# duanzhiihao/myDetection

Measured on AMD Instinct MI355X. Metric: images/sec at batch 32, 640x640, YOLOv3-80 (backbone -> FPN -> head -> decode -> NMS), higher is better.
Workload: dtype f32; 1 GPU; yolov3_80 (Darknet-53 + YOLOv3 FPN/head + decode + conf 0.005/top-512/NMS 0.45), batch 32/GPU, 640x640, random-init calibrated weights, hipGraph replay (1 batch lane per GPU); global_batch=32, image_size=640, parallelism=dp1, batch_lanes=1, batch_lanes_rule=model.batch_lanes_hint, passes=153, exchange=none

## Files before the change

include/mydet.h:

```cpp
#ifndef MYDET_H
#define MYDET_H

#include <stdint.h>

#ifdef __cplusplus
extern "C" {
#endif

#define MYDET_ABI_VERSION 2

#define MYDET_E_BADARG   (-1)
#define MYDET_E_UNSUPP   (-2)

#define MYDET_ACT_NONE   0
#define MYDET_ACT_LEAKY  1
#define MYDET_ACT_SWISH  2

int mydet_abi_version(void);

int mydet_conv2d_igemm_f32(const float *x, int64_t ldx, const float *w,
                           const float *scale, const float *shift,
                           const float *residual, int64_t ldr, const float *a_gate,
                           void *workspace, int64_t workspace_bytes,
                           float *y, int64_t ldy,
// ... 25 lines not shown
int mydet_dwconv_se_groups(int Ho, int Wo, int C, int K, int stride);
int mydet_dwconv_f32(const float *x, int64_t ldx, const float *w, const float *scale, const float *shift,
                     float *y, int64_t ldy, int B, int H, int W, int C, int K, int stride, int pad_t, int pad_l,
                     int Ho, int Wo, int act, float *se_partial, int S, const mydet_se_tail *se, void *stream);

int mydet_channel_sums_f32(const float *x, int64_t ldx, int B, int H, int W, int C, float *partial, int S,
                           void *stream);

int mydet_se_gate_f32(float *partial, int S, int B, int HW, int C, const float *w1, const float *b1, int Cse,
                      const float *w2t, const float *b2, float *gate, void *stream);

int mydet_maxpool3s2_f32(const float *x, int64_t ldx, float *y, int64_t ldy, int B, int H, int W, int C,
                         int Ho, int Wo, void *stream);

int mydet_bifpn_fuse_f32(int n, const float *in0, int64_t ld0, int mode0, const float *in1, int64_t ld1, int mode1,
                         const float *in2, int64_t ld2, int mode2, const float *weights, float *y, int64_t ldy,
                         int B, int H, int W, int C, void *stream);

int mydet_upsample_concat_f32(const float *a, int64_t lda, int Ha, int Wa, int C1,
                              const float *b, int64_t ldb, int C2,
                              float *y, int64_t ldy, int B, int Ho, int Wo, void *stream);

int mydet_conv1x1_upcat_f32(const float *x_lo, int64_t ld_lo, int C_lo, const float *x_hi, int64_t ld_hi, int C_hi,
                            const float *w, const float *scale, const float *shift, void *workspace,
                            int64_t workspace_bytes, float *y, int64_t ldy, int B, int H, int W, int Cout, int act,
                            void *stream);

int64_t mydet_split_bf16_elems(int Cout, int K);
int mydet_split_bf16_f32(const float *w, int Cout, int K, uint16_t *planes, void *stream);
int mydet_conv2d_igemm_b3_f32(const float *x, int64_t ldx, const uint16_t *w_planes, const float *scale, const float *shift,
                              const float *residual, int64_t ldr, const float *a_gate, void *workspace, int64_t workspace_bytes, float *y,
                              int64_t ldy, int B, int H, int W, int Cin, int Cout, int KH, int KW, int stride, int pad_t,
                              int pad_l, int Ho, int Wo, int act, void *stream);
int mydet_conv3x3_p3_f32(const float *x, int64_t ldx, const uint16_t *w_planes, const float *scale, const float *shift,
                         const float *residual, int64_t ldr, float *y, int64_t ldy, int B, int H, int W, int Cin, int Cout,
                         int stride, int act, void *stream);
int mydet_conv3x3_p3_plan(int Ho, int Wo, int Cout, int stride, int32_t *out);
int mydet_conv_stem_p3_f32(const float *x, int64_t sxb, int64_t sxc, int64_t sxh, int64_t sxw, const uint16_t *w0_planes,
                           const float *scale0, const float *shift0, int act0, const uint16_t *w1_planes, const float *scale1,
                           const float *shift1, int act1, float *y, int64_t ldy, int B, int H, int W, int C0, int Cout,
                           int stride0, int pad_t, int pad_l, int Hs, int Ws, int stride1, void *stream);
int mydet_conv_stem_p3_lds_bytes(void);
int mydet_conv_b3_reload_tuning(void);

int mydet_conv_igemm_occupancy(int cfg, int *assumed);

int mydet_conv_igemm_plan(int cfg, int B, int Ho, int Wo, int Cin, int Cout, int taps,
                          int64_t workspace_bytes, int cus, int32_t *out);

int mydet_space_to_depth_f32(const float *x, int64_t sb, int64_t sc, int64_t sh, int64_t sw, float *y, int64_t ldy,
                             int B, int C, int H, int W, void *stream);

int mydet_spp_concat_f32(const float *x, int64_t ldx, float *y, int64_t ldy, int B, int H, int W, int C, int k0, int k1,
                         int k2, void *stream);

#define MYDET_DECODE_YOLO   0
#define MYDET_DECODE_RETINA 1
#define MYDET_DECODE_FCOS   2
#define MYDET_DECODE_RAPID  3
typedef struct mydet_decode_level {
    const float *box; int64_t ldbox;
    const float *cls; int64_t ldcls;
    const float *anchors_wh;
    int H, W;
    float stride;
    int64_t n_off;
// ... 179 lines not shown
```

mydetection_amd/_lib.py:

```python
import ctypes
import os

_HERE = os.path.dirname(os.path.abspath(__file__))
LIB_PATH = os.environ.get('MYDET_LIB_PATH') or os.path.join(_HERE, 'lib', 'libmydet_hip.so')

c_int, c_i64, c_f32, c_f64, c_ptr = ctypes.c_int, ctypes.c_int64, ctypes.c_float, ctypes.c_double, ctypes.c_void_p

SIGNATURES = {
    'mydet_abi_version': [],
    'mydet_conv2d_igemm_f32': [c_ptr, c_i64, c_ptr, c_ptr, c_ptr, c_ptr, c_i64, c_ptr, c_ptr, c_i64, c_ptr, c_i64]
    + [c_int] * 13 + [c_ptr],
    'mydet_wino_weights_floats': [c_int, c_int],
    'mydet_wino_weights_f32': [c_ptr, c_int, c_int, c_ptr, c_ptr],
    'mydet_conv2d_wino_f32': [c_ptr, c_i64, c_ptr, c_ptr, c_ptr, c_ptr, c_i64, c_ptr, c_i64, c_ptr, c_i64] + [c_int] * 6
    + [c_ptr],
    'mydet_wino4_weights_floats': [c_int, c_int],
    'mydet_wino4_weights_f32': [c_ptr, c_int, c_int, c_ptr, c_ptr],
    'mydet_wino4_workspace_bytes': [c_int, c_int, c_int, c_int, c_int],
    'mydet_wino4_reload_tuning': [],
    'mydet_conv_b3_reload_tuning': [],
    'mydet_conv_igemm_occupancy': [c_int, c_ptr],
    'mydet_conv_igemm_plan': [c_int] * 7 + [c_i64, c_int, c_ptr],
    'mydet_split_bf16_elems': [c_int, c_int],
    'mydet_split_bf16_f32': [c_ptr, c_int, c_int, c_ptr, c_ptr],
    'mydet_conv2d_igemm_b3_f32': [c_ptr, c_i64, c_ptr, c_ptr, c_ptr, c_ptr, c_i64, c_ptr, c_ptr, c_i64, c_ptr, c_i64] + [c_int] * 13 + [c_ptr],
    'mydet_conv3x3_p3_f32': [c_ptr, c_i64, c_ptr, c_ptr, c_ptr, c_ptr, c_i64, c_ptr, c_i64] + [c_int] * 7 + [c_ptr],
    'mydet_conv3x3_p3_plan': [c_int, c_int, c_int, c_int, c_ptr],
    'mydet_conv_stem_p3_f32': [c_ptr, c_i64, c_i64, c_i64, c_i64, c_ptr, c_ptr, c_ptr, c_int, c_ptr, c_ptr, c_ptr, c_int, c_ptr, c_i64]
    + [c_int] * 11 + [c_ptr],
    'mydet_conv_stem_p3_lds_bytes': [],
    'mydet_wino4_tail_plan': [c_int, c_int, c_int, c_int, c_int, c_int, c_ptr],
    'mydet_conv2d_wino4_f32': [c_ptr, c_i64, c_ptr, c_ptr, c_ptr, c_ptr, c_i64, c_ptr, c_i64, c_ptr, c_i64] + [c_int] * 6 + [c_ptr],
    'mydet_dwconv_slices': [c_int, c_int, c_int, c_int, c_int],
    'mydet_dwconv_se_groups': [c_int, c_int, c_int, c_int, c_int],
    'mydet_dwconv_f32': [c_ptr, c_i64, c_ptr, c_ptr, c_ptr, c_ptr, c_i64] + [c_int] * 11 + [c_ptr, c_int, c_ptr, c_ptr],
    'mydet_channel_sums_f32': [c_ptr, c_i64, c_int, c_int, c_int, c_int, c_ptr, c_int, c_ptr],
    'mydet_se_gate_f32': [c_ptr, c_int, c_int, c_int, c_int, c_ptr, c_ptr, c_int, c_ptr, c_ptr, c_ptr, c_ptr],
    'mydet_maxpool3s2_f32': [c_ptr, c_i64, c_ptr, c_i64] + [c_int] * 6 + [c_ptr],
    'mydet_bifpn_fuse_f32': [c_int, c_ptr, c_i64, c_int, c_ptr, c_i64, c_int, c_ptr, c_i64, c_int, c_ptr, c_ptr, c_i64,
                             c_int, c_int, c_int, c_int, c_ptr],
    'mydet_conv2d_stem_f32': [c_ptr, c_i64, c_i64, c_i64, c_i64, c_ptr, c_ptr, c_ptr, c_ptr, c_i64] + [c_int] * 10 + [c_ptr],
    'mydet_upsample_concat_f32': [c_ptr, c_i64, c_int, c_int, c_int, c_ptr, c_i64, c_int, c_ptr, c_i64, c_int, c_int,
                                  c_int, c_ptr],
    'mydet_conv1x1_upcat_f32': [c_ptr, c_i64, c_int, c_ptr, c_i64, c_int, c_ptr, c_ptr, c_ptr, c_ptr, c_i64, c_ptr, c_i64]
    + [c_int] * 5 + [c_ptr],
    'mydet_space_to_depth_f32': [c_ptr, c_i64, c_i64, c_i64, c_i64, c_ptr, c_i64, c_int, c_int, c_int, c_int, c_ptr],
    'mydet_spp_concat_f32': [c_ptr, c_i64, c_ptr, c_i64] + [c_int] * 7 + [c_ptr],
    'mydet_decode_levels_f32': [c_int, c_int, c_ptr, c_int, c_int, c_int, c_int, c_int, c_int, c_int, c_int, c_int, c_int,
                                c_ptr, c_ptr, c_ptr, c_i64, c_ptr],
    'mydet_decode_uv5_levels_f32': [c_int, c_ptr, c_int, c_int, c_int, c_int, c_int, c_int, c_int, c_int, c_int, c_int,
                                    c_ptr, c_ptr, c_ptr, c_i64, c_ptr],
    'mydet_decode_f32': [c_int, c_ptr, c_i64, c_int, c_int, c_ptr, c_i64, c_int, c_int, c_int, c_ptr, c_int, c_int,
                         c_int, c_int, c_int, c_f32, c_int, c_int, c_ptr, c_ptr, c_ptr, c_i64, c_i64, c_ptr],
    'mydet_postprocess_f32': [c_ptr, c_ptr, c_ptr, c_int, c_i64, c_f32, c_f64, c_int, c_ptr, c_ptr, c_ptr, c_ptr,
                              c_ptr, c_ptr, c_ptr],
    'mydet_postprocess_records_f32': [c_ptr, c_ptr, c_ptr, c_int, c_i64, c_f32, c_f64, c_ptr, c_ptr, c_ptr],
    'mydet_postprocess_rot_f32': [c_ptr, c_ptr, c_ptr, c_int, c_i64, c_f32, c_f64, c_int, c_ptr, c_ptr, c_ptr, c_ptr,
                                  c_ptr, c_ptr, c_ptr],
    'mydet_postprocess_records_rot_f32': [c_ptr, c_ptr, c_ptr, c_int, c_i64, c_f32, c_f64, c_ptr, c_ptr, c_ptr],
    'mydet_postprocess_rotnms_f32': [c_ptr, c_ptr, c_ptr, c_int, c_i64, c_f32, c_f64, c_int, c_ptr, c_ptr, c_ptr, c_ptr,
                                     c_ptr, c_ptr, c_ptr],
    'mydet_postprocess_records_rotnms_f32': [c_ptr, c_ptr, c_ptr, c_int, c_i64, c_f32, c_f64, c_ptr, c_ptr, c_ptr],
    'mydet_rotated_iou_f32': [c_ptr, c_i64, c_ptr, c_i64, c_ptr, c_ptr],
    'mydet_mbconv_tiles': [c_int, c_int, c_int],
    'mydet_mbconv_expand_dw_f32': [c_ptr, c_i64, c_ptr, c_ptr, c_ptr, c_ptr, c_ptr, c_i64] + [c_int] * 11 + [c_ptr, c_int, c_ptr, c_ptr],
    'mydet_sepconv_nodes_f32': [c_int, c_ptr, c_int, c_int, c_ptr],
    'mydet_stem_dw_f32': [c_ptr, c_i64, c_i64, c_i64, c_i64, c_ptr, c_ptr, c_ptr, c_ptr, c_ptr, c_i64, c_int, c_int, c_int, c_int,
                          c_int, c_int, c_int, c_int, c_ptr, c_int, c_ptr, c_ptr],
    'mydet_lr_tb_levels_f32': [c_int, c_ptr, c_int, c_int, c_ptr],
    'mydet_sepconv_decode_retina_f32': [c_int, c_ptr, c_int, c_int, c_int, c_int, c_int, c_int, c_ptr, c_ptr, c_ptr, c_i64, c_ptr],
    'mydet_bboxes_iou_f32': [c_ptr, c_int, c_ptr, c_int, c_int, c_ptr, c_ptr],
    'mydet_bboxes_to_original_batched_f32': [c_ptr, c_i64, c_ptr, c_i64, c_int, c_int, c_ptr, c_ptr],
    'mydet_detections_to_json_f64': [c_ptr, c_i64, c_ptr, c_i64, c_ptr, c_i64, c_ptr, c_i64, c_int, c_int, c_ptr, c_int, c_ptr, c_ptr, c_ptr],
    'mydet_resize_bilinear_u8': [c_ptr, c_int, c_int, c_i64, c_ptr, c_int, c_int, c_i64, c_ptr, c_ptr, c_int, c_ptr, c_ptr, c_int, c_ptr],
    'mydet_preprocess_u8_f32': [c_ptr, c_int, c_int, c_int, c_ptr, c_int, c_int, c_int, c_ptr, c_ptr, c_ptr],
    'mydet_frames_to_input_f32': [c_ptr, c_int, c_int, c_int, c_i64, c_i64, c_ptr, c_int, c_int, c_int, c_int, c_int, c_int,
                                  c_ptr, c_ptr, c_int, c_ptr, c_ptr, c_int, c_int, c_ptr, c_ptr, c_ptr],
# ... 107 lines not shown
```

mydetection_amd/csrc/conv_igemm.hip:

```cpp
#include <cstdlib>

#include "common.h"
#include "split_bf16.h"

namespace {

constexpr unsigned OOB = 0xFFFFFFFFu;

struct ConvArgs {
    const float *x, *w, *scale, *shift, *res, *gate;
    float *y;
    int64_t ldx, ldr, ldy;
    int B, H, W, Cin, Cout, KH, KW, stride, pad_t, pad_l, Ho, Wo, act;
    int M, K, ntiles, nblk;
    int tile0, splits;
    float *ws;
    size_t ws_bytes;
    const float *x1;
    int64_t ldx1;
    int C1;
    const unsigned short *wsplit;
};

typedef unsigned u32x4 __attribute__((ext_vector_type(4)));
// ... 231 lines not shown
            store_slab(buf ^ 1, areg[d], breg[d]);
            load_slab(kt + d + 1 + PF, areg[d], breg[d]);
            __syncthreads();
            buf ^= 1;
        }
    }

    if (SPLIT) {
        constexpr int NV4 = TM * TN * 4;
        f32x4 *dst = reinterpret_cast<f32x4 *>(p.ws) + (int64_t)blockIdx.x * NV4 * NT + tid;
#pragma unroll
        for (int i = 0; i < TM; ++i)
#pragma unroll
            for (int j = 0; j < TN; ++j)
#pragma unroll
                for (int v = 0; v < 4; ++v)
                    dst[((i * TN + j) * 4 + v) * NT] =
                        f32x4{acc[i][j][4 * v], acc[i][j][4 * v + 1], acc[i][j][4 * v + 2], acc[i][j][4 * v + 3]};
        return;
    }
    const int m_base = m0 + wm * TM * 32, n_base = n0 + wn * TN * 32;
    if ((m0 + BM <= p.M) && (n0 + BN <= p.Cout))
        epilogue<ACT, RES, true, TM, TN>(p, acc, m_base, n_base, fr, fh, pscl, psft);
    else
        epilogue<ACT, RES, false, TM, TN>(p, acc, m_base, n_base, fr, fh, pscl, psft);
}

constexpr int B3_COUT_PAD = 256;
__device__ __host__ __forceinline__ int b3_unit(int rr, int h) { return 2 * rr + (h ^ ((rr >> 2) & 1)); }

#ifndef B3_PF
#define B3_PF 2
#endif
template <int BM, int BN, int ACT, bool RES, bool SPLIT = false, int PF = B3_PF, int WN = 2, bool GATE = false>
__global__ __launch_bounds__(128 * WN, 2) void conv_igemm_b3_kernel(const ConvArgs p) {
    constexpr int NT = 128 * WN, WM = 2, BK = 16;
    constexpr int ROWB = 32;
    constexpr int TM = BM / (WM * 32), TN = BN / (WN * 32);
    constexpr int AI = BM * 4 / NT;
    constexpr int BCH = BN * 2;
    constexpr int PLANE_A = BM * ROWB, PLANE_B = BN * ROWB, BUF = 3 * (PLANE_A + PLANE_B);
    extern __shared__ __attribute__((aligned(16))) char smem_b3[];

    const int tid = threadIdx.x;
    const int lid = SPLIT ? p.tile0 + (int)blockIdx.x / p.splits : mydet_xcd_remap(blockIdx.x, p.nblk);
    const int m0 = (lid / p.ntiles) * BM;
    const int n0 = (lid % p.ntiles) * BN;
    const int hwo = p.Ho * p.Wo;
    const int b0 = m0 / hwo;
    const int64_t img = (int64_t)p.H * p.W * p.ldx;
    const __amdgpu_buffer_rsrc_t xr = mydet_rsrc(p.x + b0 * img, (p.B - b0) * img * 4);
    const int CoutP = (p.Cout + B3_COUT_PAD - 1) / B3_COUT_PAD * B3_COUT_PAD;
    const __amdgpu_buffer_rsrc_t wr = mydet_rsrc(p.wsplit, (int64_t)((p.K + 15) >> 4) * 3 * CoutP * 32);

    constexpr int RP = NT / 4;
    const int sc = tid & 3, sr = tid >> 2;
    const int ntaps = p.KH * p.KW;
    int aoff[AI];
    unsigned amask[AI];
    unsigned goff[AI];
    const __amdgpu_buffer_rsrc_t gr = mydet_rsrc(GATE ? p.gate : p.x, (int64_t)p.B * p.Cin * 4);
    const bool flat = ntaps == 1 && p.stride == 1 && p.pad_t == 0 && p.pad_l == 0 && p.Ho == p.H && p.Wo == p.W;
#pragma unroll
    for (int i = 0; i < AI; ++i) {
        const int m = m0 + sr + RP * i;
        const int mm = m < p.M ? m : p.M - 1;
        goff[i] = GATE ? (unsigned)((mm / hwo) * p.Cin + sc * 4) * 4u : 0u;
        if (flat) {
            aoff[i] = (int)(((int64_t)(mm - b0 * hwo) * p.ldx + sc * 4) * 4);
            amask[i] = m < p.M ? 1u : 0u;
            continue;
        }
        const int ow = mm % p.Wo, t = mm / p.Wo;
        const int oh = t % p.Ho, b = t / p.Ho;
        const int ih0 = oh * p.stride - p.pad_t, iw0 = ow * p.stride - p.pad_l;
        aoff[i] = (int)((((int64_t)(b - b0) * p.H + ih0) * p.W + iw0) * p.ldx + sc * 4) * 4;
        unsigned mask = 0;
        for (int tp = 0; tp < ntaps; ++tp) {
            const int kh = tp / p.KW, kw = tp - kh * p.KW;
            if ((unsigned)(ih0 + kh) < (unsigned)p.H && (unsigned)(iw0 + kw) < (unsigned)p.W) mask |= 1u << tp;
        }
        amask[i] = m < p.M ? mask : 0u;
    }
    const bool bact = tid < BCH;
    const int bu = tid & 63, brr = bu >> 1;
    const int br = (tid >> 6) * 32 + brr, bh = (bu & 1) ^ ((brr >> 2) & 1);
    const unsigned boff = bact ? (unsigned)(n0 * 32 + tid * 16) : OOB;
    const unsigned plane_bytes = (unsigned)CoutP * 32u, slab_bytes = 3u * plane_bytes;

    f32x4 areg[PF][AI];
    u32x4 breg[PF][3];
    const int nk_all = (p.K + BK - 1) / BK;
    int kt0 = 0, nk = nk_all;
    if (SPLIT) {
        const int sp = (int)blockIdx.x % p.splits;
        kt0 = (int)((unsigned)(nk_all * sp) / (unsigned)p.splits);
        nk = (int)((unsigned)(nk_all * (sp + 1)) / (unsigned)p.splits);
    }
    int tap = 0, c0 = 0, tapoff = 0;
    if (SPLIT) {
        const int k0 = kt0 * BK;
        tap = k0 / p.Cin;
        c0 = k0 - tap * p.Cin;
        const int kh = tap / p.KW, kw = tap - kh * p.KW;
        tapoff = (int)(((int64_t)kh * p.W + kw) * p.ldx) * 4;
    }
    auto load_slab = [&](int kt, f32x4 (&ar)[AI], u32x4 (&brg)[3]) {
        const unsigned uoff = (unsigned)(tapoff + c0 * 4);
#pragma unroll
        for (int i = 0; i < AI; ++i) {
            bool ok = ((amask[i] >> tap) & 1u) && c0 + sc * 4 < p.Cin;
            ar[i] = buf_load16(xr, ok ? (unsigned)aoff[i] + uoff : OOB);
            if (GATE) {
                const f32x4 gv = buf_load16(gr, ok ? goff[i] + (unsigned)c0 * 4u : OOB);
#pragma unroll
                for (int e = 0; e < 4; ++e) ar[i][e] *= gv[e];
            }
        }
        c0 += BK;
        if (c0 == p.Cin) {
            c0 = 0;
            ++tap;
            const int kh = tap / p.KW, kw = tap - kh * p.KW;
            tapoff = (int)(((int64_t)kh * p.W + kw) * p.ldx) * 4;
        }
#pragma unroll
        for (int pl = 0; pl < 3; ++pl)
            brg[pl] = __builtin_amdgcn_raw_buffer_load_b128(wr, kt < nk_all ? boff : OOB,
                                                            __builtin_amdgcn_readfirstlane((unsigned)kt * slab_bytes + (unsigned)pl * plane_bytes), 0);
    };
    auto store_slab = [&](int buf, const f32x4 (&ar)[AI], const u32x4 (&brg)[3]) {
        char *a = smem_b3 + buf * BUF, *b = a + 3 * PLANE_A;
#pragma unroll
        for (int i = 0; i < AI; ++i) {
            bf16x4 q0, q1, q2;
            split3(ar[i], q0, q1, q2);
            char *d = a + (sr + RP * i) * ROWB + (((sc >> 1) ^ ((sr >> 3) & 1)) * 16) + (sc & 1) * 8;
            *reinterpret_cast<bf16x4 *>(d) = q0;
            *reinterpret_cast<bf16x4 *>(d + PLANE_A) = q1;
            *reinterpret_cast<bf16x4 *>(d + 2 * PLANE_A) = q2;
        }
        if (bact) {
#pragma unroll
            for (int pl = 0; pl < 3; ++pl) *reinterpret_cast<u32x4 *>(b + pl * PLANE_B + br * ROWB + ((bh ^ ((br >> 3) & 1)) * 16)) = brg[pl];
        }
// ... 420 lines not shown
    const TilePlan pl = plan_tiles(a.M, a.Cout, a.K, BM, BN, BK, slots, a0.ws ? a0.ws_bytes : 0);
    a.ntiles = pl.ntiles;
    const int total = pl.total, rem = pl.rem, splits = pl.splits;
    const bool split = pl.split;
    const size_t lds = (size_t)2 * (BM + BN) * (BK + 4) * sizeof(float);
    const bool cin = (a.Cin % BK) == 0;
    a.tile0 = 0; a.splits = 1;
    a.nblk = split ? total - rem : total;
    int rc = 0;
    if (a.x1) {
        if (!(BM == 64 && BN == 64 && BK == 32) || !cin || a.act != MYDET_ACT_LEAKY || a.res || a.gate) return MYDET_E_UNSUPP;
        if (a.nblk > 0) rc = launch_inst<64, 64, 2, 2, 32, true, MYDET_ACT_LEAKY, false, false, false, true>(a, lds, stream);
        if (rc || !split) return rc;
        a.tile0 = total - rem; a.splits = splits; a.nblk = rem * splits;
        rc = launch_inst<64, 64, 2, 2, 32, true, MYDET_ACT_NONE, false, false, true, true>(a, lds, stream);
        if (rc) return rc;
        return launch_fixup_act<BM, BN, WM, WN>(a, rem, stream);
    }
    if (a.nblk > 0)
        rc = cin ? launch_act<BM, BN, WM, WN, BK, true>(a, lds, stream) : launch_act<BM, BN, WM, WN, BK, false>(a, lds, stream);
    if (rc || !split) return rc;
    a.tile0 = total - rem; a.splits = splits; a.nblk = rem * splits;
    if (a.gate) {
        if (cin) rc = launch_inst<BM, BN, WM, WN, BK, true, MYDET_ACT_NONE, false, true, true>(a, lds, stream);
        else rc = launch_inst<BM, BN, WM, WN, BK, false, MYDET_ACT_NONE, false, true, true>(a, lds, stream);
    } else {
        if (cin) rc = launch_inst<BM, BN, WM, WN, BK, true, MYDET_ACT_NONE, false, false, true>(a, lds, stream);
        else rc = launch_inst<BM, BN, WM, WN, BK, false, MYDET_ACT_NONE, false, false, true>(a, lds, stream);
    }
    if (rc) return rc;
    return launch_fixup_act<BM, BN, WM, WN>(a, rem, stream);
}

template <int BM, int BN, int ACT, bool RES, bool SPLIT, int PF = B3_PF, int WN = 2, bool GATE = false>
int launch_b3_inst(const ConvArgs &a, hipStream_t stream) {
    auto kern = &conv_igemm_b3_kernel<BM, BN, ACT, RES, SPLIT, PF, WN, GATE>;
    constexpr int lds = 2 * 3 * (BM + BN) * 32;
    static unsigned long long attr_set = 0;
    if (const int e = mydet_lds_opt_in(attr_set, kern, lds)) return e;
    hipLaunchKernelGGL(kern, dim3(a.nblk), dim3(128 * WN), lds, stream, a);
    return mydet_launch_status();
}

template <int BM, int BN, int WN = 2>
int launch_b3(const ConvArgs &a0, hipStream_t stream) {
    ConvArgs a = a0;
    const int slots = 2 * mydet_cu_count();
    const int mtiles = (a.M + BM - 1) / BM;
    a.ntiles = (a.Cout + BN - 1) / BN;
    const int total = mtiles * a.ntiles;
    const int nk = (a.K + 15) / 16;
    const int rounds = total / slots;
    const int rem = total % slots;
    const bool small = rounds == 0 && total * 4 <= slots && nk >= 32;
    int splits = rem > 0 ? slots / rem : 0;
    if (splits > 16) splits = 16;
    if (splits > nk / 8) splits = nk / 8;
    const size_t need = (size_t)rem * (splits > 0 ? splits : 0) * BM * BN * sizeof(float);
    const bool split = rem > 0 && splits >= 2 && a0.ws && need <= a0.ws_bytes &&
                       (small || (nk >= 64 && rounds >= 2 && rounds <= 4 && rem * 2 <= slots));
    a.tile0 = 0; a.splits = 1;
    a.nblk = split ? total - rem : total;
    const bool res = a.res != nullptr;
    int rc = 0;
    if (a.gate) {
        if (a.act != MYDET_ACT_NONE || WN != 2) return MYDET_E_UNSUPP;
        if (a.nblk > 0)
            rc = res ? launch_b3_inst<BM, BN, MYDET_ACT_NONE, true, false, B3_PF, 2, true>(a, stream)
                     : launch_b3_inst<BM, BN, MYDET_ACT_NONE, false, false, B3_PF, 2, true>(a, stream);
        if (rc || !split) return rc;
        a.tile0 = total - rem; a.splits = splits; a.nblk = rem * splits;
        rc = launch_b3_inst<BM, BN, MYDET_ACT_NONE, false, true, B3_PF, 2, true>(a, stream);
        if (rc) return rc;
        return launch_fixup_act<BM, BN, 2, WN>(a, rem, stream);
    }
    if (a.nblk > 0) {
        switch (a.act) {
            case MYDET_ACT_LEAKY: rc = res ? launch_b3_inst<BM, BN, MYDET_ACT_LEAKY, true, false, (WN == 4 ? 2 : B3_PF), WN>(a, stream) : launch_b3_inst<BM, BN, MYDET_ACT_LEAKY, false, false, (WN == 4 ? 2 : B3_PF), WN>(a, stream); break;
            case MYDET_ACT_SWISH: rc = res ? launch_b3_inst<BM, BN, MYDET_ACT_SWISH, true, false, (WN == 4 ? 2 : B3_PF), WN>(a, stream) : launch_b3_inst<BM, BN, MYDET_ACT_SWISH, false, false, (WN == 4 ? 2 : B3_PF), WN>(a, stream); break;
            default: rc = res ? launch_b3_inst<BM, BN, MYDET_ACT_NONE, true, false, (WN == 4 ? 2 : B3_PF), WN>(a, stream) : launch_b3_inst<BM, BN, MYDET_ACT_NONE, false, false, (WN == 4 ? 2 : B3_PF), WN>(a, stream); break;
        }
    }
    if (rc || !split) return rc;
    a.tile0 = total - rem; a.splits = splits; a.nblk = rem * splits;
    rc = launch_b3_inst<BM, BN, MYDET_ACT_NONE, false, true, (WN == 4 ? 2 : B3_PF), WN>(a, stream);
    if (rc) return rc;
    return launch_fixup_act<BM, BN, 2, WN>(a, rem, stream);
}

template <int ACT, bool RES, bool SPLIT>
int launch_b3w_inst(const ConvArgs &a, hipStream_t stream) {
    auto kern = &conv_igemm_b3w_kernel<ACT, RES, SPLIT>;
    constexpr int lds = 2 * 3 * 128 * 48 + 3 * 3 * 256 * 32;
    static unsigned long long attr_set = 0;
    if (const int e = mydet_lds_opt_in(attr_set, kern, lds)) return e;
    hipLaunchKernelGGL(kern, dim3(a.nblk), dim3(512), lds, stream, a);
    return mydet_launch_status();
// ... 157 lines not shown
        return 0;
    });
}

extern "C" int64_t mydet_split_bf16_elems(int Cout, int K) {
    if (Cout <= 0 || K <= 0 || (K & 3)) return 0;
    return (int64_t)((K + 15) >> 4) * 3 * ((Cout + B3_COUT_PAD - 1) / B3_COUT_PAD * B3_COUT_PAD) * 16;
}

extern "C" int mydet_split_bf16_f32(const float *w, int Cout, int K, uint16_t *planes, void *stream) {
    if (!w || !planes || Cout <= 0 || K <= 0) return MYDET_E_BADARG;
    if (K & 3) return MYDET_E_UNSUPP;
    const int CoutP = (Cout + B3_COUT_PAD - 1) / B3_COUT_PAD * B3_COUT_PAD;
    const int64_t total = (int64_t)((K + 15) >> 4) * CoutP * 16;
    if ((total + 255) / 256 > 0x7fffffff) return MYDET_E_UNSUPP;
    hipLaunchKernelGGL(split_bf16_kernel, dim3((unsigned)((total + 255) / 256)), dim3(256), 0, (hipStream_t)stream, w, Cout, K,
                       CoutP, planes);
    return mydet_launch_status();
}

static int g_b3_form = -1;
static int b3_form() {
    if (g_b3_form < 0) {
        const char *w = getenv("MYDET_B3_WIDE"), *v = getenv("MYDET_B3_WAVES");
        g_b3_form = ((w && *w == '1') ? 1 : 0) | ((v && atoi(v) == 8) ? 2 : 0);
    }
    return g_b3_form;
}
extern "C" int mydet_conv_b3_reload_tuning(void) {
    g_b3_form = -1;
    return b3_form();
}

extern "C" int mydet_conv2d_igemm_b3_f32(const float *x, int64_t ldx, const uint16_t *w_planes, const float *scale,
                                         const float *shift, const float *residual, int64_t ldr, const float *a_gate, void *workspace,
                                         int64_t workspace_bytes, float *y, int64_t ldy, int B, int H, int W, int Cin, int Cout,
                                         int KH, int KW, int stride, int pad_t, int pad_l, int Ho, int Wo, int act, void *stream) {
    if (!x || !w_planes || !y || B <= 0 || H <= 0 || W <= 0 || Cin <= 0 || Cout <= 0 || KH <= 0 || KW <= 0 || stride <= 0 ||
        Ho <= 0 || Wo <= 0)
        return MYDET_E_BADARG;
    if ((ldx & 3) || ldx < Cin || ldy < Cout || (residual && ldr < Cout)) return MYDET_E_BADARG;
    if (((uintptr_t)x & 15) || ((uintptr_t)w_planes & 15) || ((uintptr_t)y & 15) || (residual && ((uintptr_t)residual & 15)) ||
        (scale && ((uintptr_t)scale & 15)) || (shift && ((uintptr_t)shift & 15)))
        return MYDET_E_BADARG;
    if (act < 0 || act > 2) return MYDET_E_BADARG;
    if (a_gate && (KH != 1 || KW != 1 || ((uintptr_t)a_gate & 15))) return MYDET_E_BADARG;
    if (((Cin & 15) && !(KH == 1 && KW == 1 && !(Cin & 3))) || (ldy & 3) || (residual && (ldr & 3))) return MYDET_E_UNSUPP;
    if ((Cin & 15) && (Cout > 192 ? b3_form() & 1 : 0)) return MYDET_E_UNSUPP;
    const int64_t M64 = (int64_t)B * Ho * Wo, K64 = (int64_t)KH * KW * Cin;
    if (M64 > (int64_t)1 << 30 || K64 > (int64_t)1 << 30) return MYDET_E_BADARG;
    const int64_t img_bytes = (int64_t)H * W * ldx * 4;
    const int64_t span_imgs = 256 / ((int64_t)Ho * Wo) + 2;
    if (M64 * ldy * 4 >= 0x7FFFFFF0ll || (residual && M64 * ldr * 4 >= 0x7FFFFFF0ll)) return MYDET_E_UNSUPP;
    if (KH * KW > 31 || img_bytes * span_imgs >= 0x7FFFFFF0ll || mydet_split_bf16_elems(Cout, (int)K64) * 2 >= 0x7FFFFFF0ll) return MYDET_E_UNSUPP;
    ConvArgs a;
    a.x = x; a.w = nullptr; a.scale = scale; a.shift = shift; a.res = residual; a.gate = a_gate; a.y = y;
    a.ldx = ldx; a.ldr = ldr; a.ldy = ldy;
    a.B = B; a.H = H; a.W = W; a.Cin = Cin; a.Cout = Cout; a.KH = KH; a.KW = KW; a.stride = stride;
    a.pad_t = pad_t; a.pad_l = pad_l; a.Ho = Ho; a.Wo = Wo; a.act = act;
    a.M = (int)M64; a.K = (int)K64; a.ntiles = 0; a.nblk = 0; a.tile0 = 0; a.splits = 1;
    a.x1 = nullptr; a.ldx1 = 0; a.C1 = 0; a.wsplit = w_planes;
    a.ws = ((uintptr_t)workspace & 15) ? nullptr : (float *)workspace;
    a.ws_bytes = workspace_bytes > 0 ? (size_t)workspace_bytes : 0;
    if (Cout <= 64) return launch_b3<128, 64>(a, (hipStream_t)stream);
    static const int half_tiles = [] { const char *e = getenv("MYDET_B3_HALF_TILES"); return e ? atoi(e) : mydet_cu_count() / 2; }();
    if (((M64 + 127) / 128) * ((Cout + 127) / 128) <= half_tiles) return launch_b3<64, 128>(a, (hipStream_t)stream);
    const int form = a_gate ? 0 : b3_form();
    if ((form & 1) && Cout > 192) return launch_b3w(a, (hipStream_t)stream);
    if (form & 2) return launch_b3<128, 128, 4>(a, (hipStream_t)stream);
    return launch_b3<128, 128>(a, (hipStream_t)stream);
}

extern "C" int mydet_conv_igemm_occupancy(int cfg, int *assumed) {
    int n = 0, as = 0;
    hipError_t e = hipErrorInvalidValue;
#define MYDET_OCC(BM, BN, WM, WN, BK, PER_CU)                                                                                       \
    {                                                                                                                                \
        auto kern = &conv_igemm_kernel<BM, BN, WM, WN, BK, true, MYDET_ACT_LEAKY, false, false, false, false>;                        \
        const size_t lds = (size_t)2 * (BM + BN) * (BK + 4) * sizeof(float);                                                          \
        static unsigned long long m = 0;                                                                                             \
        if (const int rc = mydet_lds_opt_in(m, kern, (int)lds)) return rc;                                                            \
        e = hipOccupancyMaxActiveBlocksPerMultiprocessor(&n, kern, WM * WN * 64, lds);                                                \
        as = PER_CU;                                                                                                                 \
    }
    switch (cfg) {
        case 0: MYDET_OCC(128, 128, 2, 2, 32, 2) break;
        case 1: MYDET_OCC(128, 64, 2, 2, 32, 2) break;
        case 2: MYDET_OCC(128, 32, 4, 1, 32, 3) break;
        case 3: MYDET_OCC(64, 64, 2, 2, 32, 4) break;
        case 6: MYDET_OCC(128, 64, 2, 2, 16, cfg6_per_cu()) break;
        case 9: MYDET_OCC(128, 96, 4, 1, 32, 2) break;
        case 8: MYDET_OCC(128, 128, 2, 4, 32, 2) break;
        default: return MYDET_E_BADARG;
    }
#undef MYDET_OCC
    if (assumed) *assumed = as;
    return e == hipSuccess ? n : MYDET_E_UNSUPP;
}

extern "C" int mydet_conv1x1_upcat_f32(const float *x_lo, int64_t ld_lo, int C_lo, const float *x_hi, int64_t ld_hi, int C_hi,
                                       const float *w, const float *scale, const float *shift, void *workspace,
                                       int64_t workspace_bytes, float *y, int64_t ldy, int B, int H, int W, int Cout, int act,
                                       void *stream) {
    if (!x_lo || !x_hi || !w || !y || B <= 0 || H <= 0 || W <= 0 || C_lo <= 0 || C_hi <= 0 || Cout <= 0) return MYDET_E_BADARG;
    if ((ld_lo & 3) || (ld_hi & 3) || ld_lo < C_lo || ld_hi < C_hi || ldy < Cout || (ldy & 3)) return MYDET_E_BADARG;
    if (((uintptr_t)x_lo & 15) || ((uintptr_t)x_hi & 15) || ((uintptr_t)w & 15) || ((uintptr_t)y & 15) ||
        (scale && ((uintptr_t)scale & 15)) || (shift && ((uintptr_t)shift & 15)))
        return MYDET_E_BADARG;
    if ((H & 1) || (W & 1) || (C_lo & 31) || (C_hi & 31) || act != MYDET_ACT_LEAKY) return MYDET_E_UNSUPP;
    const int64_t M64 = (int64_t)B * H * W;
    const int Cin = C_lo + C_hi;
    if (forced_cfg() >= 0 ? forced_cfg() != 3 : (choose_cfg(M64, Cin, Cout, 1) != 3 || (Cout <= 48 && M64 >= 65536 && pw_skinny_on())))
        return MYDET_E_UNSUPP;
    if (M64 > (int64_t)1 << 30 || M64 * ldy * 4 >= 0x7FFFFFF0ll) return MYDET_E_UNSUPP;
    const int64_t span_imgs = 256 / ((int64_t)H * W) + 2;
    if ((int64_t)H * W * ld_hi * 4 * span_imgs >= 0x7FFFFFF0ll || (int64_t)(H >> 1) * (W >> 1) * ld_lo * 4 * span_imgs >= 0x7FFFFFF0ll ||
        (int64_t)Cout * Cin * 4 >= 0x7FFFFFF0ll)
        return MYDET_E_UNSUPP;
    ConvArgs a;
    a.x = x_hi; a.w = w; a.scale = scale; a.shift = shift; a.res = nullptr; a.gate = nullptr; a.y = y;
    a.ldx = ld_hi; a.ldr = 0; a.ldy = ldy;
    a.B = B; a.H = H; a.W = W; a.Cin = Cin; a.Cout = Cout; a.KH = 1; a.KW = 1; a.stride = 1;
    a.pad_t = 0; a.pad_l = 0; a.Ho = H; a.Wo = W; a.act = act;
    a.M = (int)M64; a.K = Cin; a.ntiles = 0; a.nblk = 0;
    a.tile0 = 0; a.splits = 1;
    a.x1 = x_lo; a.ldx1 = ld_lo; a.C1 = C_lo; a.wsplit = nullptr;
    a.ws = ((uintptr_t)workspace & 15) ? nullptr : (float *)workspace;
    a.ws_bytes = workspace_bytes > 0 ? (size_t)workspace_bytes : 0;
    return launch_cfg(3, a, (hipStream_t)stream);
}
```

mydetection_amd/models/modules.py:

```python
import torch
import torch.nn as nn

from .. import ops


def _versions(*tensors):
    return tuple((t.data_ptr(), t._version) for t in tensors)


def prepare_conv(owner, slot, conv, bn, depthwise=False):
    tensors = [conv.weight] + ([bn.weight, bn.bias, bn.running_mean, bn.running_var] if bn is not None else [])
    if conv.bias is not None:
        tensors.append(conv.bias)
    key = _versions(*tensors)
    cache = owner.__dict__.setdefault('_prep_cache', {})
    hit = cache.get(slot)
    if hit is None or hit[0] != key:
        with torch.no_grad():
            w = conv.weight.detach().float()
            if depthwise:
                w = w.permute(2, 3, 0, 1).reshape(w.shape[2], w.shape[3], w.shape[0]).contiguous()
            else:
                w = w.permute(0, 2, 3, 1).contiguous()
            if bn is not None:
# ... 23 lines not shown

def prepare_b3(owner, slot, w_ohwi):
    if not ops.SPLIT_BF16 or (w_ohwi.shape[3] % 16 and not (w_ohwi.shape[1] == 1 and w_ohwi.shape[2] == 1 and w_ohwi.shape[3] % 4 == 0)):
        return None
    cache = owner.__dict__.setdefault('_prep_cache', {})
    hit = cache.get(slot)
    if hit is None or hit[0] is not w_ohwi:
        hit = (w_ohwi, ops.split_bf16(w_ohwi))
        cache[slot] = hit
    return hit[1]


class FusedConvMixin:

    def _prepared(self, conv, bn):
        return prepare_conv(self, 'main', conv, bn)


class ConvBnLeaky(nn.Module, FusedConvMixin):
    def __init__(self, c1, c2, k=1, s=1):
        super().__init__()
        self.k, self.s = k, s
        self.conv = nn.Conv2d(c1, c2, k, s, padding=(k - 1) // 2, bias=False)
        self.bn = nn.BatchNorm2d(c2, eps=1e-5, momentum=0.01)

    def forward(self, x, residual=None, upcat_lo=None):
        if self.training:
            raise NotImplementedError('mydetection_amd implements the inference path only; call model.eval()')
        w, scale, shift = self._prepared(self.conv, self.bn)
        p = (self.k - 1) // 2
        if upcat_lo is not None:
            assert residual is None
            if self.k == 1 and self.s == 1:
                y = ops.conv1x1_upcat(upcat_lo, x, w, scale, shift, ops.ACT_LEAKY)
                if y is not None:
                    return y
            x = ops.upsample_concat(upcat_lo, tuple(x.shape[2:4]), x)
        if w.shape[3] == 3 and self.k == 3 and w.shape[0] == 32 and residual is None:
            return ops.conv2d_stem(x, w, scale, shift, self.s, (p, p, p, p), ops.ACT_LEAKY)
        u, u4 = prepare_wino(self, 'wino', w) if self.k == 3 and self.s == 1 else (None, None)
        b3 = prepare_b3(self, 'b3', w) if (u is None and u4 is None) or (self.k == 3 and w.shape[3] <= ops.P3_S1_MAX_CIN) else None
        return ops.conv2d(x, w, scale, shift, self.k, self.s, (p, p, p, p), ops.ACT_LEAKY, residual=residual, wino=u, wino4=u4, b3=b3)


def stem_p3(cbl_0, cbl_1, x):
    if (cbl_0.training or cbl_1.training or (cbl_0.k, cbl_0.s, cbl_1.k, cbl_1.s) != (3, 1, 3, 2) or x.dim() != 4 or x.shape[1] != 3
            or cbl_0.conv.out_channels != 32 or cbl_1.conv.in_channels != 32 or x.dtype != torch.float32 or not x.is_cuda
            or cbl_0._forward_hooks or cbl_0._forward_pre_hooks or cbl_1._forward_hooks or cbl_1._forward_pre_hooks):
        return None
    B, _, H, W = x.shape
    if not (ops.SPLIT_BF16 and ops.stem_p3_takes(B, H, W, cbl_1.conv.out_channels, (1, 1, 1, 1))):
        return None
    w0, scale0, shift0 = cbl_0._prepared(cbl_0.conv, cbl_0.bn)
    w1, scale1, shift1 = cbl_1._prepared(cbl_1.conv, cbl_1.bn)
    cache = cbl_0.__dict__.setdefault('_prep_cache', {})
    hit = cache.get('stem_p3')
    if hit is None or hit[0] is not w0:
        hit = (w0, ops.stem_p3_weights(w0))
        cache['stem_p3'] = hit
    return ops.conv_stem_p3(x, hit[1], scale0, shift0, (1, 1, 1, 1), prepare_b3(cbl_1, 'b3', w1), scale1, shift1)


class DarkBlock(nn.Module):
    def __init__(self, in_out, hidden):
        super().__init__()
        self.cbl_0 = ConvBnLeaky(in_out, hidden, k=1, s=1)
        self.cbl_1 = ConvBnLeaky(hidden, in_out, k=3, s=1)
# ... 85 lines not shown
```

mydetection_amd/ops.py:

```python
import collections
import ctypes
import functools
import os
import threading

import numpy as np
import torch

from . import _lib

ACT_NONE, ACT_LEAKY, ACT_SWISH = 0, 1, 2
DECODE_YOLO, DECODE_RETINA, DECODE_FCOS, DECODE_RAPID = 0, 1, 2, 3
TOPK = 512


def _stream():
    return ctypes.c_void_p(torch.cuda.current_stream().cuda_stream)


class KernelTimer:

    def __init__(self, chain=False):
        self.spans = {}
        self.bytes = {}
# ... 746 lines not shown
        cout = A * n_cls if nd['kind'] == 0 else A * 4
        work += px * (2 * C + C + cout + cout) + (12.0 if nd['kind'] == 0 else 16.0) * B * A * H * W
        fused += px * C + (12.0 if nd['kind'] == 0 else 16.0) * B * A * H * W
    t0 = TIMER.start() if TIMER else None
    code = _lib.lib().mydet_sepconv_decode_retina_f32(len(nodes), ctypes.cast(arr, ctypes.c_void_p), B, C, A, n_cls,
                                                      int(img_hw[0]), int(img_hw[1]), _ptr(bbox), _ptr(class_idx),
                                                      _ptr(score), bbox.shape[1], _stream())
    if t0:
        TIMER.stop('sepconv_decode', t0, work, work, fused=fused)
    _lib.check(code, 'mydet_sepconv_decode_retina_f32')


def upsample_concat(a, size, b=None):
    require_gpu(a, 'upsample_concat')
    a, lda = to_nhwc(a)
    B, C1, Ha, Wa = a.shape
    Ho, Wo = size
    C2, ldb = 0, 0
    if b is not None:
        b, ldb = to_nhwc(b)
        C2 = b.shape[1]
        assert b.shape[0] == B and tuple(b.shape[2:]) == (Ho, Wo)
    out, ldy = empty_nhwc(B, C1 + C2, Ho, Wo, a.device)
    t0 = TIMER.start() if TIMER else None
    code = _lib.lib().mydet_upsample_concat_f32(_ptr(a), lda, Ha, Wa, C1, _ptr(b), ldb, C2, _ptr(out), ldy, B, Ho,
                                                Wo, _stream())
    if t0:
        TIMER.stop('upsample_concat', t0, *[4.0 * B * (C1 * Ha * Wa + C2 * Ho * Wo + (C1 + C2) * Ho * Wo)] * 2)
    _lib.check(code, 'mydet_upsample_concat_f32')
    return out


FUSED_UPCAT = os.environ.get('MYDET_FUSED_UPCAT', '1') != '0'


def conv1x1_upcat(a, b, w_ohwi, scale, shift, act):
    require_gpu(a, 'conv1x1_upcat')
    B, C1, Ha, Wa = a.shape
    _, C2, H, W = b.shape
    Cout = w_ohwi.shape[0]
    if not FUSED_UPCAT or (H, W) != (2 * Ha, 2 * Wa) or C1 % 32 or C2 % 32 or act != ACT_LEAKY or w_ohwi.shape[1:3] != (1, 1):
        return None
    a, lda = to_nhwc(a)
    b, ldb = to_nhwc(b)
    out, ldy = empty_nhwc(B, Cout, H, W, a.device)
    ws = conv_workspace(a.device)
    t0 = TIMER.start() if TIMER else None
    code = _lib.lib().mydet_conv1x1_upcat_f32(_ptr(a), lda, C1, _ptr(b), ldb, C2, _ptr(w_ohwi), _ptr(scale), _ptr(shift), _ptr(ws),
                                              ws.numel() * 4, _ptr(out), ldy, B, H, W, Cout, act, _stream())
    if code == -2:
        return None
    if t0:
        name = f'conv_igemm {C1}^+{C2}->{Cout} k1s1 {H}x{W}' if TIMER_DETAIL else 'conv_igemm'
        TIMER.stop(name, t0, 2.0 * B * H * W * Cout * (C1 + C2), 4.0 * (B * (Ha * Wa * C1 + H * W * C2) + B * H * W * Cout + (C1 + C2) * Cout))
    _lib.check(code, 'mydet_conv1x1_upcat_f32')
    return out


def space_to_depth(x):
    require_gpu(x, 'space_to_depth')
    assert x.dtype == torch.float32 and x.dim() == 4
    B, C, H, W = x.shape
    assert H % 2 == 0 and W % 2 == 0
    out, ldy = empty_nhwc(B, 4 * C, H // 2, W // 2, x.device)
    sb, sc, sh, sw = x.stride()
    t0 = TIMER.start() if TIMER else None
    code = _lib.lib().mydet_space_to_depth_f32(_ptr(x), sb, sc, sh, sw, _ptr(out), ldy, B, C, H, W, _stream())
    if t0:
        TIMER.stop('space_to_depth', t0, *[8.0 * B * C * H * W] * 2)
    _lib.check(code, 'mydet_space_to_depth_f32')
    return out


def spp_concat(x, ks=(5, 9, 13)):
    require_gpu(x, 'spp_concat')
    assert len(ks) == 3
    x, ldx = to_nhwc(x)
    B, C, H, W = x.shape
    assert C % 4 == 0
# ... 460 lines not shown
```

Before: 1604 images/sec.

## Fuse nearest-upsample concat into the split-bf16 b3 1x1 conv kernel

Adds a CAT template mode to the b3 (three-plane bf16 split) implicit-GEMM kernel. The first C1 input channels are read straight from the low-resolution tensor at (oh/2, ow/2), and the rest come from the high-resolution tensor. The YOLOv3 FPN upsample+concat+1x1 conv then runs on the tensor-core b3 path instead of the older fused f32 upcat kernel. This avoids materialising the concatenated tensor and uses the faster matrix path, at the cost of a per-slab branch and an extra buffer resource in the loader.

```diff
diff --git a/include/mydet.h b/include/mydet.h
--- a/include/mydet.h
+++ b/include/mydet.h
@@ -81,6 +81,10 @@
                               const float *residual, int64_t ldr, const float *a_gate, void *workspace, int64_t workspace_bytes, float *y,
                               int64_t ldy, int B, int H, int W, int Cin, int Cout, int KH, int KW, int stride, int pad_t,
                               int pad_l, int Ho, int Wo, int act, void *stream);
+int mydet_conv1x1_upcat_b3_f32(const float *x_lo, int64_t ld_lo, int C_lo, const float *x_hi, int64_t ld_hi, int C_hi,
+                               const uint16_t *w_planes, const float *scale, const float *shift, void *workspace,
+                               int64_t workspace_bytes, float *y, int64_t ldy, int B, int H, int W, int Cout, int act,
+                               void *stream);
 int mydet_conv3x3_p3_f32(const float *x, int64_t ldx, const uint16_t *w_planes, const float *scale, const float *shift,
                          const float *residual, int64_t ldr, float *y, int64_t ldy, int B, int H, int W, int Cin, int Cout,
                          int stride, int act, void *stream);
diff --git a/mydetection_amd/_lib.py b/mydetection_amd/_lib.py
--- a/mydetection_amd/_lib.py
+++ b/mydetection_amd/_lib.py
@@ -43,6 +43,8 @@
     'mydet_upsample_concat_f32': [c_ptr, c_i64, c_int, c_int, c_int, c_ptr, c_i64, c_int, c_ptr, c_i64, c_int, c_int,
                                   c_int, c_ptr],
     'mydet_conv1x1_upcat_f32': [c_ptr, c_i64, c_int, c_ptr, c_i64, c_int, c_ptr, c_ptr, c_ptr, c_ptr, c_i64, c_ptr, c_i64]
+    + [c_int] * 5 + [c_ptr],
+    'mydet_conv1x1_upcat_b3_f32': [c_ptr, c_i64, c_int, c_ptr, c_i64, c_int, c_ptr, c_ptr, c_ptr, c_ptr, c_i64, c_ptr, c_i64]
     + [c_int] * 5 + [c_ptr],
     'mydet_space_to_depth_f32': [c_ptr, c_i64, c_i64, c_i64, c_i64, c_ptr, c_i64, c_int, c_int, c_int, c_int, c_ptr],
     'mydet_spp_concat_f32': [c_ptr, c_i64, c_ptr, c_i64] + [c_int] * 7 + [c_ptr],
diff --git a/mydetection_amd/csrc/conv_igemm.hip b/mydetection_amd/csrc/conv_igemm.hip
--- a/mydetection_amd/csrc/conv_igemm.hip
+++ b/mydetection_amd/csrc/conv_igemm.hip
@@ -287,7 +287,7 @@
 #ifndef B3_PF
 #define B3_PF 2
 #endif
-template <int BM, int BN, int ACT, bool RES, bool SPLIT = false, int PF = B3_PF, int WN = 2, bool GATE = false>
+template <int BM, int BN, int ACT, bool RES, bool SPLIT = false, int PF = B3_PF, int WN = 2, bool GATE = false, bool CAT = false>
 __global__ __launch_bounds__(128 * WN, 2) void conv_igemm_b3_kernel(const ConvArgs p) {
     constexpr int NT = 128 * WN, WM = 2, BK = 16;
     constexpr int ROWB = 32;
@@ -305,6 +305,8 @@
     const int b0 = m0 / hwo;
     const int64_t img = (int64_t)p.H * p.W * p.ldx;
     const __amdgpu_buffer_rsrc_t xr = mydet_rsrc(p.x + b0 * img, (p.B - b0) * img * 4);
+    const int64_t img1 = (int64_t)(p.H >> 1) * (p.W >> 1) * p.ldx1;
+    const __amdgpu_buffer_rsrc_t xr1 = mydet_rsrc(CAT ? p.x1 + b0 * img1 : p.x, CAT ? (p.B - b0) * img1 * 4 : 16);
     const int CoutP = (p.Cout + B3_COUT_PAD - 1) / B3_COUT_PAD * B3_COUT_PAD;
     const __amdgpu_buffer_rsrc_t wr = mydet_rsrc(p.wsplit, (int64_t)((p.K + 15) >> 4) * 3 * CoutP * 32);
 
@@ -314,6 +316,7 @@
     int aoff[AI];
     unsigned amask[AI];
     unsigned goff[AI];
+    unsigned aoff1[AI];
     const __amdgpu_buffer_rsrc_t gr = mydet_rsrc(GATE ? p.gate : p.x, (int64_t)p.B * p.Cin * 4);
     const bool flat = ntaps == 1 && p.stride == 1 && p.pad_t == 0 && p.pad_l == 0 && p.Ho == p.H && p.Wo == p.W;
 #pragma unroll
@@ -321,6 +324,11 @@
         const int m = m0 + sr + RP * i;
         const int mm = m < p.M ? m : p.M - 1;
         goff[i] = GATE ? (unsigned)((mm / hwo) * p.Cin + sc * 4) * 4u : 0u;
+        if (CAT) {
+            const int ow = mm % p.W, t = mm / p.W;
+            const int oh = t % p.H, b = t / p.H;
+            aoff1[i] = (unsigned)((((int64_t)(b - b0) * (p.H >> 1) + (oh >> 1)) * (p.W >> 1) + (ow >> 1)) * p.ldx1 + sc * 4) * 4u;
+        }
         if (flat) {
             aoff[i] = (int)(((int64_t)(mm - b0 * hwo) * p.ldx + sc * 4) * 4);
             amask[i] = m < p.M ? 1u : 0u;
@@ -361,11 +369,13 @@
         tapoff = (int)(((int64_t)kh * p.W + kw) * p.ldx) * 4;
     }
     auto load_slab = [&](int kt, f32x4 (&ar)[AI], u32x4 (&brg)[3]) {
-        const unsigned uoff = (unsigned)(tapoff + c0 * 4);
+        const bool lo = CAT && c0 < p.C1;
+        const unsigned uoff = (unsigned)(tapoff + (c0 - (CAT && !lo ? p.C1 : 0)) * 4);
 #pragma unroll
         for (int i = 0; i < AI; ++i) {
             bool ok = ((amask[i] >> tap) & 1u) && c0 + sc * 4 < p.Cin;
-            ar[i] = buf_load16(xr, ok ? (unsigned)aoff[i] + uoff : OOB);
+            if (CAT) ar[i] = buf_load16(lo ? xr1 : xr, ok ? (lo ? aoff1[i] : (unsigned)aoff[i]) + uoff : OOB);
+            else ar[i] = buf_load16(xr, ok ? (unsigned)aoff[i] + uoff : OOB);
             if (GATE) {
                 const f32x4 gv = buf_load16(gr, ok ? goff[i] + (unsigned)c0 * 4u : OOB);
 #pragma unroll
@@ -852,9 +862,9 @@
     return launch_fixup_act<BM, BN, WM, WN>(a, rem, stream);
 }
 
-template <int BM, int BN, int ACT, bool RES, bool SPLIT, int PF = B3_PF, int WN = 2, bool GATE = false>
+template <int BM, int BN, int ACT, bool RES, bool SPLIT, int PF = B3_PF, int WN = 2, bool GATE = false, bool CAT = false>
 int launch_b3_inst(const ConvArgs &a, hipStream_t stream) {
-    auto kern = &conv_igemm_b3_kernel<BM, BN, ACT, RES, SPLIT, PF, WN, GATE>;
+    auto kern = &conv_igemm_b3_kernel<BM, BN, ACT, RES, SPLIT, PF, WN, GATE, CAT>;
     constexpr int lds = 2 * 3 * (BM + BN) * 32;
     static unsigned long long attr_set = 0;
     if (const int e = mydet_lds_opt_in(attr_set, kern, lds)) return e;
@@ -883,6 +893,18 @@
     a.nblk = split ? total - rem : total;
     const bool res = a.res != nullptr;
     int rc = 0;
+    if (a.x1) {
+        if constexpr (WN == 2) {
+            if (a.act != MYDET_ACT_LEAKY || res || a.gate) return MYDET_E_UNSUPP;
+            if (a.nblk > 0) rc = launch_b3_inst<BM, BN, MYDET_ACT_LEAKY, false, false, B3_PF, 2, false, true>(a, stream);
+            if (rc || !split) return rc;
+            a.tile0 = total - rem; a.splits = splits; a.nblk = rem * splits;
+            rc = launch_b3_inst<BM, BN, MYDET_ACT_NONE, false, true, B3_PF, 2, false, true>(a, stream);
+            if (rc) return rc;
+            return launch_fixup_act<BM, BN, 2, WN>(a, rem, stream);
+        }
+        return MYDET_E_UNSUPP;
+    }
     if (a.gate) {
         if (a.act != MYDET_ACT_NONE || WN != 2) return MYDET_E_UNSUPP;
         if (a.nblk > 0)
@@ -1106,6 +1128,11 @@
     return b3_form();
 }
 
+static int b3_half_tiles() {
+    static const int v = [] { const char *e = getenv("MYDET_B3_HALF_TILES"); return e ? atoi(e) : mydet_cu_count() / 2; }();
+    return v;
+}
+
 extern "C" int mydet_conv2d_igemm_b3_f32(const float *x, int64_t ldx, const uint16_t *w_planes, const float *scale,
                                          const float *shift, const float *residual, int64_t ldr, const float *a_gate, void *workspace,
                                          int64_t workspace_bytes, float *y, int64_t ldy, int B, int H, int W, int Cin, int Cout,
@@ -1137,8 +1164,7 @@
     a.ws = ((uintptr_t)workspace & 15) ? nullptr : (float *)workspace;
     a.ws_bytes = workspace_bytes > 0 ? (size_t)workspace_bytes : 0;
     if (Cout <= 64) return launch_b3<128, 64>(a, (hipStream_t)stream);
-    static const int half_tiles = [] { const char *e = getenv("MYDET_B3_HALF_TILES"); return e ? atoi(e) : mydet_cu_count() / 2; }();
-    if (((M64 + 127) / 128) * ((Cout + 127) / 128) <= half_tiles) return launch_b3<64, 128>(a, (hipStream_t)stream);
+    if (((M64 + 127) / 128) * ((Cout + 127) / 128) <= b3_half_tiles()) return launch_b3<64, 128>(a, (hipStream_t)stream);
     const int form = a_gate ? 0 : b3_form();
     if ((form & 1) && Cout > 192) return launch_b3w(a, (hipStream_t)stream);
     if (form & 2) return launch_b3<128, 128, 4>(a, (hipStream_t)stream);
@@ -1203,3 +1229,35 @@
     a.ws_bytes = workspace_bytes > 0 ? (size_t)workspace_bytes : 0;
     return launch_cfg(3, a, (hipStream_t)stream);
 }
+
+extern "C" int mydet_conv1x1_upcat_b3_f32(const float *x_lo, int64_t ld_lo, int C_lo, const float *x_hi, int64_t ld_hi, int C_hi,
+                                          const uint16_t *w_planes, const float *scale, const float *shift, void *workspace,
+                                          int64_t workspace_bytes, float *y, int64_t ldy, int B, int H, int W, int Cout, int act,
+                                          void *stream) {
+    if (!x_lo || !x_hi || !w_planes || !y || B <= 0 || H <= 0 || W <= 0 || C_lo <= 0 || C_hi <= 0 || Cout <= 0) return MYDET_E_BADARG;
+    if ((ld_lo & 3) || (ld_hi & 3) || ld_lo < C_lo || ld_hi < C_hi || ldy < Cout || (ldy & 3)) return MYDET_E_BADARG;
+    if (((uintptr_t)x_lo & 15) || ((uintptr_t)x_hi & 15) || ((uintptr_t)w_planes & 15) || ((uintptr_t)y & 15) ||
+        (scale && ((uintptr_t)scale & 15)) || (shift && ((uintptr_t)shift & 15)))
+        return MYDET_E_BADARG;
+    if ((H & 1) || (W & 1) || (C_lo & 15) || (C_hi & 15) || act != MYDET_ACT_LEAKY) return MYDET_E_UNSUPP;
+    if (Cout <= 64 || b3_form()) return MYDET_E_UNSUPP;
+    const int64_t M64 = (int64_t)B * H * W;
+    const int Cin = C_lo + C_hi;
+    if (M64 > (int64_t)1 << 30 || M64 * ldy * 4 >= 0x7FFFFFF0ll) return MYDET_E_UNSUPP;
+    const int64_t span_imgs = 256 / ((int64_t)H * W) + 2;
+    if ((int64_t)H * W * ld_hi * 4 * span_imgs >= 0x7FFFFFF0ll || (int64_t)(H >> 1) * (W >> 1) * ld_lo * 4 * span_imgs >= 0x7FFFFFF0ll ||
+        mydet_split_bf16_elems(Cout, Cin) * 2 >= 0x7FFFFFF0ll)
+        return MYDET_E_UNSUPP;
+    ConvArgs a;
+    a.x = x_hi; a.w = nullptr; a.scale = scale; a.shift = shift; a.res = nullptr; a.gate = nullptr; a.y = y;
+    a.ldx = ld_hi; a.ldr = 0; a.ldy = ldy;
+    a.B = B; a.H = H; a.W = W; a.Cin = Cin; a.Cout = Cout; a.KH = 1; a.KW = 1; a.stride = 1;
+    a.pad_t = 0; a.pad_l = 0; a.Ho = H; a.Wo = W; a.act = act;
+    a.M = (int)M64; a.K = Cin; a.ntiles = 0; a.nblk = 0;
+    a.tile0 = 0; a.splits = 1;
+    a.x1 = x_lo; a.ldx1 = ld_lo; a.C1 = C_lo; a.wsplit = w_planes;
+    a.ws = ((uintptr_t)workspace & 15) ? nullptr : (float *)workspace;
+    a.ws_bytes = workspace_bytes > 0 ? (size_t)workspace_bytes : 0;
+    if (((M64 + 127) / 128) * ((Cout + 127) / 128) <= b3_half_tiles()) return launch_b3<64, 128>(a, (hipStream_t)stream);
+    return launch_b3<128, 128>(a, (hipStream_t)stream);
+}
diff --git a/mydetection_amd/models/modules.py b/mydetection_amd/models/modules.py
--- a/mydetection_amd/models/modules.py
+++ b/mydetection_amd/models/modules.py
@@ -79,7 +79,7 @@
         if upcat_lo is not None:
             assert residual is None
             if self.k == 1 and self.s == 1:
-                y = ops.conv1x1_upcat(upcat_lo, x, w, scale, shift, ops.ACT_LEAKY)
+                y = ops.conv1x1_upcat(upcat_lo, x, w, scale, shift, ops.ACT_LEAKY, b3=prepare_b3(self, 'b3', w))
                 if y is not None:
                     return y
             x = ops.upsample_concat(upcat_lo, tuple(x.shape[2:4]), x)
diff --git a/mydetection_amd/ops.py b/mydetection_amd/ops.py
--- a/mydetection_amd/ops.py
+++ b/mydetection_amd/ops.py
@@ -802,19 +802,38 @@
 
 
 FUSED_UPCAT = os.environ.get('MYDET_FUSED_UPCAT', '1') != '0'
-
-
-def conv1x1_upcat(a, b, w_ohwi, scale, shift, act):
+UPCAT_B3 = os.environ.get('MYDET_UPCAT_B3', '1') != '0'
+
+
+def upcat_b3_takes(M, C1, C2, Cout):
+    return UPCAT_B3 and C1 % 16 == 0 and C2 % 16 == 0 and b3_takes(M, C1 + C2, Cout, 1)
+
+
+def conv1x1_upcat(a, b, w_ohwi, scale, shift, act, b3=None):
     require_gpu(a, 'conv1x1_upcat')
     B, C1, Ha, Wa = a.shape
     _, C2, H, W = b.shape
     Cout = w_ohwi.shape[0]
-    if not FUSED_UPCAT or (H, W) != (2 * Ha, 2 * Wa) or C1 % 32 or C2 % 32 or act != ACT_LEAKY or w_ohwi.shape[1:3] != (1, 1):
+    if not FUSED_UPCAT or (H, W) != (2 * Ha, 2 * Wa) or act != ACT_LEAKY or w_ohwi.shape[1:3] != (1, 1):
+        return None
+    use_b3 = b3 is not None and upcat_b3_takes(B * H * W, C1, C2, Cout)
+    if not use_b3 and (C1 % 32 or C2 % 32):
         return None
     a, lda = to_nhwc(a)
     b, ldb = to_nhwc(b)
     out, ldy = empty_nhwc(B, Cout, H, W, a.device)
     ws = conv_workspace(a.device)
+    if use_b3:
+        t0 = TIMER.start() if TIMER else None
+        code = _lib.lib().mydet_conv1x1_upcat_b3_f32(_ptr(a), lda, C1, _ptr(b), ldb, C2, _ptr(b3), _ptr(scale), _ptr(shift), _ptr(ws),
+                                                     ws.numel() * 4, _ptr(out), ldy, B, H, W, Cout, act, _stream())
+        if code == -2:
+            return None
+        if t0:
+            name = f'conv_igemm_b3 {C1}^+{C2}->{Cout} k1s1 {H}x{W}' if TIMER_DETAIL else 'conv_igemm_b3'
+            TIMER.stop(name, t0, 2.0 * B * H * W * Cout * (C1 + C2), 4.0 * (B * (Ha * Wa * C1 + H * W * C2) + B * H * W * Cout + (C1 + C2) * Cout))
+        _lib.check(code, 'mydet_conv1x1_upcat_b3_f32')
+        return out
     t0 = TIMER.start() if TIMER else None
     code = _lib.lib().mydet_conv1x1_upcat_f32(_ptr(a), lda, C1, _ptr(b), ldb, C2, _ptr(w_ohwi), _ptr(scale), _ptr(shift), _ptr(ws),
                                               ws.numel() * 4, _ptr(out), ldy, B, H, W, Cout, act, _stream())
```

Measured after the change: 1617 images/sec (median of 6 runs). About the same (+0.8%).
